# METHODS-Group/ProximalGalerkin

Measured on AMD Instinct MI355X. Metric: proximal-Newton iterations/sec, 2048^2 P1 obstacle (LVPP Newton inner loop), higher is better.
Workload: dtype f64; 1 GPU; 2048x2048 right-diagonal P1 obstacle problem on [-1,1]^2, phi_set obstacle, f=0, settings B: alpha double_exponential, alpha_max 100, tol 0.0001; snes_rtol 1e-6, Newton linear solves to true relative residual 1e-10; mixed_unknowns=8396802, step=one full LVPP solve from the zero state, parallelism=single

## Files before the change

proximalgalerkin_amd/csrc/pgx_api.hip:

```cpp
#include <algorithm>
#include <atomic>
#include <chrono>
#include <thread>
#include <cmath>
#include <cstdio>
#include <cstring>
#include <deque>
#include <map>
#include <mutex>
#include <string>
#include <vector>

#include "../../include/pgx.h"
#include "../../include/pgx_nd.h"
#include "pgx_comm.h"
#include "pgx_internal.h"

static thread_local std::string g_create_error;

struct DistLevel {
  int g, glo, H, ghi;
};
struct Dist {
  bool on = false;
// ... 105 lines not shown
  int xcd_remap = 2;
  int tail_verts = 1100;
  int spmv_stream = 1;
  int nu_coarse = 0;
  int fused_k3 = 1;
  int fused_legs = 1;
  int fused_min = 4000;
  int cgs_selective = 1;
  long cgs_skipped = 0, cgs_total = 0;
  double cgs_eta2 = 1e-4;
  TailArgs tail{};
  pgx_nd* lu = nullptr;
  pgx_comm* lu_comm = nullptr;
  double* Jmix = nullptr;
  bool dh_interior = false;
  int stag_its = 12;
  double stag_gain = 1e-4;
  int smooth_d32 = 0;
  int k6_max = 0;
  int mg_f32 = 1;
  int f32_min = 4000;
  int f32_k6_max = 4300000;
  int f32_rr_max = 300000;
  int resid_grid = 1;
  int spmv_stencil = 1;
  bool lu_active = false;
  bool check_replicas = false;
  double *obs_partials = nullptr, *d_out6 = nullptr;
  int obs_blocks = 0;
  bool prof = false;
// ... 978 lines not shown
  if (!h->patch_f32) h->patch_sym = 0;
  if (h->patch_f32 == 2 && !h->patch_sym) h->patch_f32 = 1;
  if (const char* e = pgx_tune("PGX_P2_FALLBACK_ITS")) h->p2_fallback_its = std::max(1, atoi(e));
  {
    const char* e = pgx_tune("PGX_TAIL2");
    pgxk_mg_tail_select(e ? atoi(e) : 1);
  }
  if (const char* e = pgx_tune("PGX_FUSED_LEGS")) h->fused_legs = atoi(e);
  if (const char* e = pgx_tune("PGX_FUSED_K3")) h->fused_k3 = atoi(e);
  if (const char* e = pgx_tune("PGX_NU_COARSE")) h->nu_coarse = atoi(e);
  if (const char* e = pgx_tune("PGX_SPMV_STREAM")) h->spmv_stream = atoi(e);
  if (const char* e = pgx_tune("PGX_SPMV_BAL")) h->spmv_bal = atoi(e);
  if (const char* e = pgx_tune("PGX_SPMV_DICT")) h->spmv_dict = atoi(e);
  if (const char* e = pgx_tune("PGX_SPMV_STENCIL")) h->spmv_stencil = atoi(e);
  if (const char* e = pgx_tune("PGX_RESID_GRID")) h->resid_grid = atoi(e);
  if (const char* e = pgx_tune("PGX_K6_MAX")) h->k6_max = atoi(e);
  if (const char* e = pgx_tune("PGX_SMOOTH_D32")) h->smooth_d32 = atoi(e);
  if (const char* e = pgx_tune("PGX_HOST_POLL")) h->host_poll = atoi(e);
  if (const char* e = pgx_tune("PGX_GS_WIDE")) h->gs_wide = atoi(e) >= 16 ? 16 : 8;
  if (const char* e = pgx_tune("PGX_FUSED_PUBLISH")) h->fused_publish = atoi(e);
  if (const char* e = pgx_tune("PGX_FUSED_RESID")) h->fused_resid = atoi(e);
  if (const char* e = pgx_tune("PGX_LEAN_RHS")) h->lean_rhs = atoi(e);
  if (const char* e = pgx_tune("PGX_FUSED_STEP")) h->fused_step = atoi(e);
  if (const char* e = pgx_tune("PGX_LAZY_NORM")) h->lazy_norm = atoi(e);
  if (const char* e = pgx_tune("PGX_V_F32")) h->v_f32 = atoi(e);
  if (const char* e = pgx_tune("PGX_V_F32_GAIN")) h->v_f32_gain = atof(e);
  if (const char* e = pgx_tune("PGX_V_F32_MAX")) h->v_f32_max = atof(e);
  if (const char* e = pgx_tune("PGX_V_F32_MIN")) h->v_f32_min = atoi(e);
  if (const char* e = pgx_tune("PGX_Z_F32")) h->z_f32 = atoi(e);
  if (const char* e = pgx_tune("PGX_F32_DBF16")) h->f32_dbf16 = atoi(e);
// ... 501 lines not shown
    const int rc = allreduce_dev(h, h->d_small, 1);
    if (rc) return rc;
  }
  {
    const int rc = replica_agree(h, h->d_small, 1);
    if (rc) return rc;
  }
  {
    const int rc = fetch_small(h, h->d_small, 1);
    if (rc) return rc;
  }
  *out = std::sqrt(h->h_small[0]);
  return PGX_OK;
}

static void residual_dev(pgx_handle* h, const double* x, double* F, int with_d = 0) {
  PhaseTimer t(h, 0);
  if (h->degree == 2) {
    pgxk_residual_p2_cells(h->st, h->nc, h->nd, h->cdofs, h->coords, h->mask, h->gbc, x, h->xk, h->alpha, h->f, h->q2,
                           h->p2_v2c_ptr, h->p2_v2c_ent, h->p2_stash, F, h->geoq);
    pgxk_residual_final(h->st, h->nd, h->mask, h->gbc, h->bphi, x, F);
    return;
  }
  if (h->resid_grid && h->structured && !h->lev.empty() && h->lev[0].uniform) {
    pgxk_resid_fill_grid(h->st, with_d ? 1 : 0, h->lev[0], h->fill_lds, h->rowptr, h->v2c_ptr, h->v2c_ent, h->v2c_pos, h->cells,
                         h->coords, h->mask, h->gbc, h->bphi, x, h->xk, h->alpha, h->f, h->q, F, h->Dv, with_d);
    h->dh_interior = with_d != 0;
    if (with_d == 2) h->dv_lean = true;
    if (with_d == 1) h->dv_lean = false;
    return;
  }
  pgxk_resid_fill_p1(h->st, with_d, h->n, h->fill_lds, h->rowptr, h->v2c_ptr, h->v2c_ent, h->v2c_pos, h->cells,
                     h->coords, h->mask, h->gbc, h->bphi, x, h->xk, h->alpha, h->f, h->q, F, h->Dv, h->geoq);
}

static int jacobian_dev(pgx_handle* h, const double* x, bool have_d = false) {
  if (!(have_d && h->degree == 1)) {
    PhaseTimer t(h, 1);
    if (h->degree == 2) {
      pgxk_fill_rows_p2(h->st, 2, h->nd, h->s_fill_lds, h->s_rowptr, h->p2_v2c_ptr, h->p2_v2c_ent, h->p2_v2c_pos,
                        h->cdofs, h->coords, x + h->nd, h->q2, h->s_D, h->geoq);
      pgxk_fill_rows_p1_Dp2(h->st, h->n, h->fill_lds, h->rowptr, h->v2c_ptr, h->v2c_ent, h->v2c_pos, h->cdofs, h->coords,
                            x + h->nd, h->q2, h->Dv, h->geoq);
    } else if (h->resid_grid && h->structured && !h->lev.empty() && h->lev[0].uniform) {
      pgxk_resid_fill_grid(h->st, 1, h->lev[0], h->fill_lds, h->rowptr, h->v2c_ptr, h->v2c_ent, h->v2c_pos, h->cells, h->coords,
                           h->mask, h->gbc, h->bphi, x, h->xk, h->alpha, h->f, h->q, h->w, h->Dv, 1);
      h->dh_interior = true;
      h->dv_lean = false;
      have_d = true;
    } else {
      pgxk_fill_rows(h->st, 2, h->n, h->fill_lds, h->rowptr, h->v2c_ptr, h->v2c_ent, h->v2c_pos, h->cells, h->coords,
                     x + h->n, h->q, h->Dv, h->geoq);
    }
  }
  if (h->structured) {
    PhaseTimer t(h, 2);
    pgxk_csr_to_stencil_h(h->st, h->n, h->nx + 1, h->rowptr, h->colm, h->Dv, h->lev[0].Dh,
                          (have_d && h->degree == 1 && h->dh_interior) ? h->lev[0].ny : 0);
    h->dh_interior = false;
    if (h->lev[0].Dh32) pgxk_to_float(h->st, (size_t)4 * h->n, h->lev[0].Dh, h->lev[0].Dh32);
    if (h->lev[0].f32) pgxk_f_pack_d(h->st, h->lev[0]);
    if (h->lev[0].Dd4) pgxk_pack_d4(h->st, h->lev[0]);
    const int ld = h->dist.on ? h->dist.ldist : 0;
    for (size_t l = 1; l < h->lev.size(); ++l) {
      if (h->dist.on && (int)l == ld) {
        const Dist& D = h->dist;
        const GridLevel& G = h->lev[l];
#ifdef PGX_DSTEN_FLOAT
        h->err = "PGX_DSTEN_FLOAT builds do not support sharded handles";
        return PGX_EINVAL;
#else
        pgxk_rap7h(h->st, h->lev[l - 1], h->lev[l - 1].Dh, D.view, D.view_S);
        pgxk_view_to_global(h->st, 4, D.view.n, G.n, G.nx + 1, D.view_row0, D.view_own0, D.view_H, D.view_S, G.Dh);
        const int rc = allreduce_dev(h, G.Dh, (size_t)4 * G.n);
        if (rc) return rc;
#endif
      } else {
        pgxk_rap7h(h->st, h->lev[l - 1], h->lev[l - 1].Dh, h->lev[l], h->lev[l].Dh);
      }
      if (h->lev[l].f32) pgxk_f_pack_d(h->st, h->lev[l]);
    }
  }
  h->jac_valid = true;
  h->patch_fresh = false;
  h->p2st.fresh = false;
  return PGX_OK;
}

static bool p2st_ready(pgx_handle* h) {
  pgx_handle::P2St& S = h->p2st;
  if (S.state == 0 || !S.select || (h->dist.on && !S.dist_enable) || !h->s_K || !h->s_D) return false;
  static const int nt[4] = {19, 9, 9, 9}, off[4] = {0, 19, 28, 37};
  const size_t G = (size_t)h->n;
// ... 1464 lines not shown
```

proximalgalerkin_amd/csrc/pgx_internal.h:

```cpp
#pragma once
#include <hip/hip_runtime.h>
#include <stdint.h>
#include <stddef.h>

#include "pgx_scope.h"

#ifdef PGX_DSTEN_FLOAT
typedef float dsten_t;
#else
typedef double dsten_t;
#endif

#define PGX_MAX_NQ 16
#define PGX_BLOCK 256
#ifndef PGX_TILE_X
#define PGX_TILE_X 32
#define PGX_TILE_Y 16
#endif
#ifndef PGX_ROWMAP_TY
#define PGX_ROWMAP_TY 16
#endif
#ifndef PGX_ROWMAP_BLOCK
#define PGX_ROWMAP_BLOCK 512
#endif
// ... 18 lines not shown
  double *xu, *xp, *xu2, *xp2;
  double *bu, *bp;
  double *ru, *rp;
  int f32;
  double4* Dd4;
  void* Dq;
  int dbf16;
  float2 *xf, *xf2, *bf;
};

struct StConst {
  double K[7], M[7];
  int uniform;
};

#define PGX_TAIL_MAX 8
#define PGX_TAIL_VERTS 17000
struct TailLevel {
  int nx, ny, n;
  int interior_free;
  double ic[8];
  const double *K, *M;
  const dsten_t* Dh;
  StConst sc;
  const uint8_t* mask;
  double *xu, *xp, *xu2, *xp2, *bu, *bp, *ru, *rp;
};
struct TailArgs {
  int nlev, nu, coarse_sweeps;
  double alpha, omega;
// ... 33 lines not shown
                       double* out, const PgxDotScale* scale = nullptr, int wide = 8);
int pgxk_multidot_blocks(size_t len);
int pgxk_stream_blocks(size_t len);
void pgxk_reduce_publish(hipStream_t st, int nb, const double* partials, int nrows, double* out, double* hout, int n1, const double* src1,
                         double* dst1, unsigned long long seq, unsigned long long* seqp);
int pgxk_axpy_norms(hipStream_t st, size_t len, const double* x, double* y, double* partials);
void pgxk_multiaxpy(hipStream_t st, size_t len, int nv, const double* V, size_t ldv, const double* h, double* w);
void pgxk_lincomb(hipStream_t st, size_t len, int nv, const double* Z, size_t ldz, const double* y, double* x,
                  int accumulate);

void pgxk_csr_to_stencil(hipStream_t st, int n, int sx, const int32_t* rowptr, const int32_t* colm, const double* vals,
                         double* S);
void pgxk_csr_to_stencil_h(hipStream_t st, int n, int sx, const int32_t* rowptr, const int32_t* colm,
                           const double* vals, dsten_t* Sh, int frame_ny = 0);
void pgxk_rap7(hipStream_t st, const GridLevel& f, const double* Sf, const GridLevel& c, double* Sc);
void pgxk_rap7h(hipStream_t st, const GridLevel& f, const dsten_t* Sfh, const GridLevel& c, dsten_t* Sch);
void pgxk_st_apply(hipStream_t st, int mode, const GridLevel& L, double alpha, const double* xu, const double* xp,
                   const double* bu, const double* bp, double omega, int first, double* yu, double* yp);
void pgxk_restrict(hipStream_t st, const GridLevel& f, const double* ru, const double* rp, const GridLevel& c,
                   double* bu, double* bp);
void pgxk_prolong_add(hipStream_t st, const GridLevel& c, const double* cu, const double* cp, const GridLevel& f,
                      double* xu, double* xp);
void pgxk_coarse_mask(hipStream_t st, const GridLevel& c, uint8_t* mask_c, const GridLevel& f);
void pgxk_view_to_global(hipStream_t st, int ns, int n_view, int n_glob, int sx, int row0, int own0, int nown,
                         const double* in, double* out);
void pgxk_st_smooth2(hipStream_t st, int post, const GridLevel& L, double alpha, const double* xu, const double* xp,
                     const GridLevel* C, const double* cu, const double* cp, const double* bu, const double* bp,
                     double omega, int remap, double* yu, double* yp);
void pgxk_st_spmv(hipStream_t st, const GridLevel& L, double alpha, const double* xu, const double* xp, int remap, double* yu,
                  double* yp, const float2* xf = nullptr ,
                  const double* bu = nullptr, const double* bp = nullptr, double s = 1.0 );
// ... 69 lines not shown
void pgxk_p2st_pack(hipStream_t st, int nx, int nv, int i0, int ni, int j0, int nj, size_t G, const int32_t* rowptr, const double* D,
                    void* Dst, int f32);
void pgxk_p2st_check(hipStream_t st, const P2StTab& S, int nx, int nv, int i0, int ni, int j0, int nj, double alpha_ref, double tol,
                     const int32_t* rowptr, const double* K, const double* M, int* fail);
void pgxk_p2_rows_csr(hipStream_t st, int nrows, const int32_t* rows, const int32_t* rowptr, const int32_t* colm, const double* K,
                      const double* M, const double* D, double alpha, const uint8_t* mask, const double* xu, const double* xp,
                      const double* bu, const double* bp, double* yu, double* yp);
void pgxk_resid_fill_p1(hipStream_t st, int write_d, int n, size_t lds_bytes, const int32_t* rowptr,
                        const int32_t* v2c_ptr, const int32_t* v2c_ent, const int32_t* v2c_pos, const int32_t* cells,
                        const double* coords, const uint8_t* mask, const double* gbc, const double* bphi,
                        const double* x, const double* xk, double alpha, double f, QuadTab q, double* F, double* Dout,
                        const double* geo = nullptr);
void pgxk_resid_fill_grid(hipStream_t st, int write_d, const GridLevel& L, size_t lds_bytes, const int32_t* rowptr,
                          const int32_t* v2c_ptr, const int32_t* v2c_ent, const int32_t* v2c_pos, const int32_t* cells,
                          const double* coords, const uint8_t* mask, const double* gbc, const double* bphi, const double* x,
                          const double* xk, double alpha, double f, QuadTab q, double* F, double* Dout, int write_sh);
void pgxk_axpy_dot(hipStream_t st, size_t len, int nv, const double* V, size_t ldv, const double* h1, double* w,
                   double* partials, double* out);
void pgxk_multiaxpy_scale(hipStream_t st, size_t len, int nv, const double* V, size_t ldv, const double* h,
                          double scale, double* w);
void pgxk_multiaxpy_norm(hipStream_t st, size_t len, int nv, const double* V, size_t ldv, const double* h, double* w,
                         double* partials, double* out, int wide = 8);
void pgxk_multiaxpy_norm_f32(hipStream_t st, size_t len, int nv, const float* V, size_t ldv, const double* h, int from_vnext, double* w,
                             float* vnext, double* partials, double* out, int wide = 8);
void pgxk_f_pack_d(hipStream_t st, const GridLevel& L);
void pgxk_f_smooth(hipStream_t st, int K, int first, const GridLevel& L, double alpha, const float2* xf, const double* b64u,
                   const double* b64p, const GridLevel* C, const float2* cf, const double* cdu, const double* cdp, double omega,
                   int remap, float2* yf, double* y64u, double* y64p, float2* cbf = nullptr, double* cb64u = nullptr,
                   double* cb64p = nullptr, double bscale = 1.0,
                   const float* b32u = nullptr, const float* b32p = nullptr);
void pgxk_f_resid_restrict(hipStream_t st, const GridLevel& L, double alpha, const float2* xf, const GridLevel& C, int remap,
// ... 6 lines not shown
```

proximalgalerkin_amd/csrc/pgx_kernels.hip:

```cpp
#include "pgx_internal.h"
#include "pgx_stencil.h"
#include <algorithm>
#include <type_traits>

#define WAVE 64

static bool first_use_on_device(int slot) {
  static bool done[4][64] = {};
  int dev = 0;
  if (hipGetDevice(&dev) != hipSuccess || dev < 0 || dev >= 64) return true;
  if (done[slot][dev]) return false;
  done[slot][dev] = true;
  return true;
}

__device__ __forceinline__ double wave_sum(double v) {
#pragma unroll
  for (int o = WAVE / 2; o > 0; o >>= 1) v += __shfl_xor(v, o, WAVE);
  return v;
}

__device__ __forceinline__ double2 ldnt2(const double2* p) {
  typedef double v2d __attribute__((ext_vector_type(2)));
  const v2d v = __builtin_nontemporal_load((const v2d*)p);
// ... 418 lines not shown
      for (int k = rowptr[i]; k < rowptr[i + 1]; ++k) Dout[k] = row[k - rowptr[i]];
  }
  if (WRITE_D && !FRAME) {
    __syncthreads();
    for (int k = threadIdx.x; k < len; k += PGX_BLOCK) Dout[base + k] = acc[k];
  }
}

#define PGX_RF_TX 32
#define PGX_RF_TY 12
template <bool WRITE_D>
__global__ void __launch_bounds__(PGX_RF_TX * PGX_RF_TY) k_resid_fill_grid(
    int nx, int ny, int n, const int32_t* __restrict__ rowptr, const double* __restrict__ coords, const uint8_t* __restrict__ mask,
    const double* __restrict__ gbc, const double* __restrict__ bphi, const double* __restrict__ x, const double* __restrict__ xk,
    double alpha, double f, QuadTab q, StConst sc, double* __restrict__ F, double* __restrict__ Dout,
    dsten_t* __restrict__ Sh) {
  constexpr int TX = PGX_RF_TX, TY = PGX_RF_TY, IW = TX + 2, IH = TY + 2, SW = TX + 1, SH = TY + 1;
  __shared__ double iu[IH * IW], ip[IH * IW], idp[IH * IW];
  __shared__ double E[2 * SW * SH][6];
  const int sx = nx + 1;
  const int ntx = (nx - 1 + TX - 1) / TX;
  const int i1 = 1 + ((int)blockIdx.x % ntx) * TX, j1 = 1 + ((int)blockIdx.x / ntx) * TY;
  const int tid = threadIdx.x;
  for (int t = tid; t < IH * IW; t += TX * TY) {
    const int gi = i1 - 1 + t % IW, gj = j1 - 1 + t / IW;
    double u = 0.0, p = 0.0, dp = 0.0;
    if (gi <= nx && gj <= ny) {
      const int v = gj * sx + gi;
      u = mask[v] ? gbc[v] : x[v];
      p = x[n + v];
      dp = p - xk[n + v];
// ... 46 lines not shown
      double* d = Dout + rowptr[v];
      d[0] = dSW;
      d[1] = dS;
      d[2] = dW;
      d[3] = dC;
      d[4] = dE;
      d[5] = dN;
      d[6] = dNE;
    }
    if (Sh) {
      Sh[v] = (dsten_t)dC;
      Sh[(size_t)n + v] = (dsten_t)dE;
      Sh[2 * (size_t)n + v] = (dsten_t)dN;
      Sh[3 * (size_t)n + v] = (dsten_t)dNE;
    }
  }
  const int o = (lj + 1) * IW + li + 1;
  const int off[7] = {0, 1, -1, IW, -IW, IW + 1, -IW - 1};
  double Ku = 0.0, Mdp = 0.0, Mu = 0.0;
#pragma unroll
  for (int t = 0; t < 7; ++t) {
    Ku += sc.K[t] * iu[o + off[t]];
    Mdp += sc.M[t] * idp[o + off[t]];
    Mu += sc.M[t] * iu[o + off[t]];
  }
  const double load = adet * 2.0 * (q.mref[0] + q.mref[1] + q.mref[2]);
  F[v] = mask[v] ? x[v] - gbc[v] : alpha * Ku + Mdp - alpha * f * load;
  F[n + v] = Mu - (((dSW + dS) + (dW + dC)) + ((dE + dN) + dNE)) - bphi[v];
}

void pgxk_resid_fill_p1(hipStream_t st, int write_d, int n, size_t lds_bytes, const int32_t* rowptr,
                        const int32_t* v2c_ptr, const int32_t* v2c_ent, const int32_t* v2c_pos, const int32_t* cells,
                        const double* coords, const uint8_t* mask, const double* gbc, const double* bphi,
                        const double* x, const double* xk, double alpha, double f, QuadTab q, double* F, double* Dout,
                        const double* geo) {
  dim3 grid((n + PGX_BLOCK - 1) / PGX_BLOCK), block(PGX_BLOCK);
  if (geo) {
    if (write_d)
      hipLaunchKernelGGL((k_resid_fill_p1_c<true>), grid, block, lds_bytes, st, n, rowptr, v2c_ptr, v2c_ent, v2c_pos, cells, mask, gbc,
                         bphi, x, xk, alpha, f, q, F, Dout, geo);
    else
      hipLaunchKernelGGL((k_resid_fill_p1_c<false>), grid, block, lds_bytes, st, n, rowptr, v2c_ptr, v2c_ent, v2c_pos, cells, mask, gbc,
                         bphi, x, xk, alpha, f, q, F, Dout, geo);
    return;
  }
  if (write_d)
    hipLaunchKernelGGL((k_resid_fill_p1<true, false>), grid, block, lds_bytes, st, n, rowptr, v2c_ptr, v2c_ent, v2c_pos, cells,
                       coords, mask, gbc, bphi, x, xk, alpha, f, q, 0, 0, F, Dout);
  else
    hipLaunchKernelGGL((k_resid_fill_p1<false, false>), grid, block, lds_bytes, st, n, rowptr, v2c_ptr, v2c_ent, v2c_pos, cells,
                       coords, mask, gbc, bphi, x, xk, alpha, f, q, 0, 0, F, Dout);
}

void pgxk_resid_fill_grid(hipStream_t st, int write_d, const GridLevel& L, size_t lds_bytes, const int32_t* rowptr,
                          const int32_t* v2c_ptr, const int32_t* v2c_ent, const int32_t* v2c_pos, const int32_t* cells,
                          const double* coords, const uint8_t* mask, const double* gbc, const double* bphi, const double* x,
                          const double* xk, double alpha, double f, QuadTab q, double* F, double* Dout, int write_sh) {
  const int n = L.n, sx = L.nx + 1;
  dim3 grid((n + PGX_BLOCK - 1) / PGX_BLOCK), block(PGX_BLOCK);
  if (write_d)
    hipLaunchKernelGGL((k_resid_fill_p1<true, true>), grid, block, lds_bytes, st, n, rowptr, v2c_ptr, v2c_ent, v2c_pos, cells,
                       coords, mask, gbc, bphi, x, xk, alpha, f, q, sx, L.ny, F, Dout);
  else
    hipLaunchKernelGGL((k_resid_fill_p1<false, true>), grid, block, lds_bytes, st, n, rowptr, v2c_ptr, v2c_ent, v2c_pos, cells,
                       coords, mask, gbc, bphi, x, xk, alpha, f, q, sx, L.ny, F, Dout);
  if (L.nx < 2 || L.ny < 2) return;
  const int ntx = (L.nx - 1 + PGX_RF_TX - 1) / PGX_RF_TX, nty = (L.ny - 1 + PGX_RF_TY - 1) / PGX_RF_TY;
  const StConst sc = make_stconst(L);
  if (write_d)
    hipLaunchKernelGGL(k_resid_fill_grid<true>, dim3(ntx * nty), dim3(PGX_RF_TX * PGX_RF_TY), 0, st, L.nx, L.ny, n, rowptr, coords,
                       mask, gbc, bphi, x, xk, alpha, f, q, sc, F, write_sh == 2 ? nullptr : Dout, write_sh ? L.Dh : nullptr);
  else
    hipLaunchKernelGGL(k_resid_fill_grid<false>, dim3(ntx * nty), dim3(PGX_RF_TX * PGX_RF_TY), 0, st, L.nx, L.ny, n, rowptr, coords,
                       mask, gbc, bphi, x, xk, alpha, f, q, sc, F, Dout, nullptr);
}

void pgxk_fill_rows(hipStream_t st, int mode, int n, size_t lds_bytes, const int32_t* rowptr, const int32_t* v2c_ptr,
                    const int32_t* v2c_ent, const int32_t* v2c_pos, const int32_t* cells, const double* coords,
                    const double* psi, QuadTab q, double* out, const double* geo) {
  dim3 grid((n + PGX_BLOCK - 1) / PGX_BLOCK), block(PGX_BLOCK);
  if (geo) {
    if (mode == 0)
      hipLaunchKernelGGL(k_fill_rows_c<0>, grid, block, lds_bytes, st, n, rowptr, v2c_ptr, v2c_ent, v2c_pos, cells, psi, q, out, geo);
    else if (mode == 1)
      hipLaunchKernelGGL(k_fill_rows_c<1>, grid, block, lds_bytes, st, n, rowptr, v2c_ptr, v2c_ent, v2c_pos, cells, psi, q, out, geo);
    else
      hipLaunchKernelGGL(k_fill_rows_c<2>, grid, block, lds_bytes, st, n, rowptr, v2c_ptr, v2c_ent, v2c_pos, cells, psi, q, out, geo);
    return;
  }
// ... 1110 lines not shown
    const double v = vals[k];
    if (o == 0) s[0] = v;
    else if (o == 1) s[1] = v;
    else if (o == sx) s[2] = v;
    else if (o == sx + 1) s[3] = v;
  }
#pragma unroll
  for (int k = 0; k < 4; ++k) Sh[(size_t)k * n + i] = (dsten_t)s[k];
}
void pgxk_csr_to_stencil_h(hipStream_t st, int n, int sx, const int32_t* rowptr, const int32_t* colm,
                           const double* vals, dsten_t* Sh, int frame_ny) {
  hipLaunchKernelGGL(k_csr_to_stencil_h, dim3((n + PGX_BLOCK - 1) / PGX_BLOCK), dim3(PGX_BLOCK), 0, st, n, sx, rowptr,
                     colm, vals, Sh, frame_ny);
}

__global__ void __launch_bounds__(PGX_BLOCK) k_rap7h(int nxf, int nyf, int nf, const dsten_t* __restrict__ Sfh, int nxc,
                                                     int nyc, int ncv, dsten_t* __restrict__ Sch) {
  const int C = blockIdx.x * blockDim.x + threadIdx.x;
  if (C >= ncv) return;
  constexpr int OX[7] = {0, 1, -1, 0, 0, 1, -1};
  constexpr int OY[7] = {0, 0, 0, 1, -1, 1, -1};
  constexpr int KEEP[4] = {0, 1, 3, 5};
  const int sxc = nxc + 1, sxf = nxf + 1;
  const int I = C % sxc, Jc = C / sxc;
  double out[4] = {0, 0, 0, 0};
#pragma unroll
  for (int oa = 0; oa < 7; ++oa) {
    const int ax = 2 * I + OX[oa], ay = 2 * Jc + OY[oa];
    if (ax < 0 || ax > nxf || ay < 0 || ay > nyf) continue;
    const double wa = pw(OX[oa], OY[oa]);
    const int a = ay * sxf + ax;
    double cf[7];
    ld7h(Sfh, nf, sxf, a, ax, ay, nxf, nyf, cf);
#pragma unroll
    for (int os = 0; os < 7; ++os) {
      const double coef = wa * cf[os];
      const int dx = OX[oa] + OX[os], dy = OY[oa] + OY[os];
#pragma unroll
      for (int q = 0; q < 4; ++q) {
        const double w2 = pw(dx - 2 * OX[KEEP[q]], dy - 2 * OY[KEEP[q]]);
        if (w2 != 0.0) out[q] += coef * w2;
      }
    }
  }
#pragma unroll
  for (int q = 0; q < 4; ++q) {
    const int nx_ = I + OX[KEEP[q]], ny_ = Jc + OY[KEEP[q]];
    const bool ok = nx_ >= 0 && nx_ <= nxc && ny_ >= 0 && ny_ <= nyc;
    Sch[(size_t)q * ncv + C] = (dsten_t)(ok ? out[q] : 0.0);
  }
}
void pgxk_rap7h(hipStream_t st, const GridLevel& f, const dsten_t* Sfh, const GridLevel& c, dsten_t* Sch) {
  hipLaunchKernelGGL(k_rap7h, dim3((c.n + PGX_BLOCK - 1) / PGX_BLOCK), dim3(PGX_BLOCK), 0, st, f.nx, f.ny, f.n, Sfh,
                     c.nx, c.ny, c.n, Sch);
}

__global__ void k_coarse_mask(int nxc, int nyc, int ncv, int nxf, const uint8_t* __restrict__ mf,
                              uint8_t* __restrict__ mc) {
  const int C = blockIdx.x * blockDim.x + threadIdx.x;
  if (C >= ncv) return;
  const int I = C % (nxc + 1), J = C / (nxc + 1);
  mc[C] = mf[(size_t)(2 * J) * (nxf + 1) + 2 * I];
}
void pgxk_coarse_mask(hipStream_t st, const GridLevel& c, uint8_t* mask_c, const GridLevel& f) {
  hipLaunchKernelGGL(k_coarse_mask, dim3((c.n + PGX_BLOCK - 1) / PGX_BLOCK), dim3(PGX_BLOCK), 0, st, c.nx, c.ny, c.n,
                     f.nx, f.mask, mask_c);
}

__global__ void __launch_bounds__(PGX_BLOCK) k_view_to_global(int ns, int n_view, int n_glob, int sx, int row0,
// ... 1829 lines not shown
```

proximalgalerkin_amd/csrc/pgx_mg32.hip:

```cpp
#include <algorithm>

#include "pgx_internal.h"
#include "pgx_stencil.h"

#define F32_BLOCK 512
#ifndef F32_LEAN
#define F32_LEAN 0
#endif
#ifndef F32_WAVES_EU
#define F32_WAVES_EU 2
#endif
#ifndef F32_K6_SPLIT
#define F32_K6_SPLIT 0
#endif
#ifndef F32_K6_TY_TOP
#define F32_K6_TY_TOP 20
#endif
#define F32_RR_CYB 2
#define F32_TB 2
__host__ __device__ constexpr int f32_tb(int K, int RR) { return (K == 6 && !RR) ? 4 : F32_TB; }

__device__ __forceinline__ float lane_shr1f(float x) {
  int v = __float_as_int(x);
  v = __builtin_amdgcn_update_dpp(v, v, 0x138, 0xf, 0xf, false);
  return __int_as_float(v);
}

typedef float f_v2f __attribute__((ext_vector_type(2)));
typedef __bf16 f_v2bf __attribute__((ext_vector_type(2)));
__device__ __forceinline__ uint32_t f_pack_bf16x2(float lo, float hi) {
  const f_v2f f = {lo, hi};
  return __builtin_bit_cast(uint32_t, __builtin_convertvector(f, f_v2bf));
}
__device__ __forceinline__ void f_pack_d(float4 q, float4& out) { out = q; }
__device__ __forceinline__ void f_pack_d(float4 q, uint2& out) { out = make_uint2(f_pack_bf16x2(q.x, q.y), f_pack_bf16x2(q.z, q.w)); }
__device__ __forceinline__ float4 f_unpack_d(float4 q) { return q; }
__device__ __forceinline__ float4 f_unpack_d(uint2 w) {
  return make_float4(__uint_as_float(w.x << 16), __uint_as_float(w.x & 0xffff0000u), __uint_as_float(w.y << 16),
                     __uint_as_float(w.y & 0xffff0000u));
}
__device__ __forceinline__ void f_zero_d(float4& q) { q = make_float4(0.f, 0.f, 0.f, 0.f); }
__device__ __forceinline__ void f_zero_d(uint2& w) { w = make_uint2(0u, 0u); }

template <class DT>
__global__ void __launch_bounds__(256) k_f_pack_d(int n, const dsten_t* __restrict__ Dh, DT* __restrict__ Dq) {
  const int v = blockIdx.x * blockDim.x + threadIdx.x;
  if (v >= n) return;
  const float big = 1e30f;
  f_pack_d(make_float4(fminf((float)Dh[v], big), fminf((float)Dh[(size_t)n + v], big), fminf((float)Dh[2 * (size_t)n + v], big),
                       fminf((float)Dh[3 * (size_t)n + v], big)),
           Dq[v]);
}
void pgxk_f_pack_d(hipStream_t st, const GridLevel& L) {
  if (L.dbf16)
    hipLaunchKernelGGL(k_f_pack_d<uint2>, dim3((L.n + 255) / 256), dim3(256), 0, st, L.n, L.Dh, (uint2*)L.Dq);
  else
    hipLaunchKernelGGL(k_f_pack_d<float4>, dim3((L.n + 255) / 256), dim3(256), 0, st, L.n, L.Dh, (float4*)L.Dq);
}

struct FCoef {
  float kv[7], mv[7], dv[7];
  int rowbc;
};
struct FConst {
  float kc[7], mc[7];
  float k0, k1, k3, k5, m0, m1, m3, m5;
// ... 1116 lines not shown
```

Before: 151.4 Newton iterations/s.

## Write fine-level stencil and packed copies directly from residual fill; LDS-staged RAP

When enabled (default on for structured uniform single-GPU P1), the grid residual/fill kernel writes the fine stencil Dh plus its double4 and f32/bf16 packed copies directly. A new frame-only kernel handles boundary vertices, replacing the full-mesh CSR fill pass. This skips the separate csr_to_stencil, f_pack_d and pack_d4 passes on the fine level. The Galerkin RAP kernel also emits packed coarse copies inline, and on large coarse levels stages the fine stencil in LDS tiles, removing the per-level pack launches and redundant global loads. Costs are more register and store pressure in the fused kernels and a more complex code path.

```diff
diff --git a/proximalgalerkin_amd/csrc/pgx_api.hip b/proximalgalerkin_amd/csrc/pgx_api.hip
--- a/proximalgalerkin_amd/csrc/pgx_api.hip
+++ b/proximalgalerkin_amd/csrc/pgx_api.hip
@@ -143,6 +143,9 @@
   pgx_comm* lu_comm = nullptr;
   double* Jmix = nullptr;
   bool dh_interior = false;
+  int d_direct = 1;
+  int rap_lds_min = 60000;
+  bool d0_direct = false;
   int stag_its = 12;
   double stag_gain = 1e-4;
   int smooth_d32 = 0;
@@ -1151,6 +1154,8 @@
   if (const char* e = pgx_tune("PGX_SPMV_DICT")) h->spmv_dict = atoi(e);
   if (const char* e = pgx_tune("PGX_SPMV_STENCIL")) h->spmv_stencil = atoi(e);
   if (const char* e = pgx_tune("PGX_RESID_GRID")) h->resid_grid = atoi(e);
+  if (const char* e = pgx_tune("PGX_D_DIRECT")) h->d_direct = atoi(e);
+  if (const char* e = pgx_tune("PGX_RAP_LDS_MIN")) h->rap_lds_min = atoi(e);
   if (const char* e = pgx_tune("PGX_K6_MAX")) h->k6_max = atoi(e);
   if (const char* e = pgx_tune("PGX_SMOOTH_D32")) h->smooth_d32 = atoi(e);
   if (const char* e = pgx_tune("PGX_HOST_POLL")) h->host_poll = atoi(e);
@@ -1682,6 +1687,11 @@
   return PGX_OK;
 }
 
+static bool d_direct_on(const pgx_handle* h) {
+  return h->d_direct && !h->dist.on && h->degree == 1 && h->structured && h->resid_grid && !h->lev.empty() && h->lev[0].uniform &&
+         sizeof(dsten_t) == 8 && !h->lev[0].Dh32;
+}
+
 static void residual_dev(pgx_handle* h, const double* x, double* F, int with_d = 0) {
   PhaseTimer t(h, 0);
   if (h->degree == 2) {
@@ -1692,8 +1702,9 @@
   }
   if (h->resid_grid && h->structured && !h->lev.empty() && h->lev[0].uniform) {
     pgxk_resid_fill_grid(h->st, with_d ? 1 : 0, h->lev[0], h->fill_lds, h->rowptr, h->v2c_ptr, h->v2c_ent, h->v2c_pos, h->cells,
-                         h->coords, h->mask, h->gbc, h->bphi, x, h->xk, h->alpha, h->f, h->q, F, h->Dv, with_d);
+                         h->coords, h->mask, h->gbc, h->bphi, x, h->xk, h->alpha, h->f, h->q, F, h->Dv, with_d, d_direct_on(h), h->colm);
     h->dh_interior = with_d != 0;
+    h->d0_direct = with_d != 0 && d_direct_on(h);
     if (with_d == 2) h->dv_lean = true;
     if (with_d == 1) h->dv_lean = false;
     return;
@@ -1712,8 +1723,9 @@
                             x + h->nd, h->q2, h->Dv, h->geoq);
     } else if (h->resid_grid && h->structured && !h->lev.empty() && h->lev[0].uniform) {
       pgxk_resid_fill_grid(h->st, 1, h->lev[0], h->fill_lds, h->rowptr, h->v2c_ptr, h->v2c_ent, h->v2c_pos, h->cells, h->coords,
-                           h->mask, h->gbc, h->bphi, x, h->xk, h->alpha, h->f, h->q, h->w, h->Dv, 1);
+                           h->mask, h->gbc, h->bphi, x, h->xk, h->alpha, h->f, h->q, h->w, h->Dv, 1, d_direct_on(h), h->colm);
       h->dh_interior = true;
+      h->d0_direct = d_direct_on(h);
       h->dv_lean = false;
       have_d = true;
     } else {
@@ -1723,12 +1735,16 @@
   }
   if (h->structured) {
     PhaseTimer t(h, 2);
-    pgxk_csr_to_stencil_h(h->st, h->n, h->nx + 1, h->rowptr, h->colm, h->Dv, h->lev[0].Dh,
-                          (have_d && h->degree == 1 && h->dh_interior) ? h->lev[0].ny : 0);
+    const bool direct = d_direct_on(h);
+    const bool d0 = direct && have_d && h->dh_interior && h->d0_direct;
+    if (!d0)
+      pgxk_csr_to_stencil_h(h->st, h->n, h->nx + 1, h->rowptr, h->colm, h->Dv, h->lev[0].Dh,
+                            (have_d && h->degree == 1 && h->dh_interior) ? h->lev[0].ny : 0);
     h->dh_interior = false;
+    h->d0_direct = false;
     if (h->lev[0].Dh32) pgxk_to_float(h->st, (size_t)4 * h->n, h->lev[0].Dh, h->lev[0].Dh32);
-    if (h->lev[0].f32) pgxk_f_pack_d(h->st, h->lev[0]);
-    if (h->lev[0].Dd4) pgxk_pack_d4(h->st, h->lev[0]);
+    if (h->lev[0].f32 && !d0) pgxk_f_pack_d(h->st, h->lev[0]);
+    if (h->lev[0].Dd4 && !d0) pgxk_pack_d4(h->st, h->lev[0]);
     const int ld = h->dist.on ? h->dist.ldist : 0;
     for (size_t l = 1; l < h->lev.size(); ++l) {
       if (h->dist.on && (int)l == ld) {
@@ -1744,7 +1760,8 @@
         if (rc) return rc;
 #endif
       } else {
-        pgxk_rap7h(h->st, h->lev[l - 1], h->lev[l - 1].Dh, h->lev[l], h->lev[l].Dh);
+        pgxk_rap7h(h->st, h->lev[l - 1], h->lev[l - 1].Dh, h->lev[l], h->lev[l].Dh, direct, direct && h->lev[l].n >= h->rap_lds_min);
+        if (direct) continue;
       }
       if (h->lev[l].f32) pgxk_f_pack_d(h->st, h->lev[l]);
     }
diff --git a/proximalgalerkin_amd/csrc/pgx_internal.h b/proximalgalerkin_amd/csrc/pgx_internal.h
--- a/proximalgalerkin_amd/csrc/pgx_internal.h
+++ b/proximalgalerkin_amd/csrc/pgx_internal.h
@@ -56,6 +56,20 @@
   int uniform;
 };
 
+typedef float f_v2f __attribute__((ext_vector_type(2)));
+typedef __bf16 f_v2bf __attribute__((ext_vector_type(2)));
+__device__ __forceinline__ uint32_t f_pack_bf16x2(float lo, float hi) {
+  const f_v2f f = {lo, hi};
+  return __builtin_bit_cast(uint32_t, __builtin_convertvector(f, f_v2bf));
+}
+__device__ __forceinline__ void f_pack_d(float4 q, float4& out) { out = q; }
+__device__ __forceinline__ void f_pack_d(float4 q, uint2& out) { out = make_uint2(f_pack_bf16x2(q.x, q.y), f_pack_bf16x2(q.z, q.w)); }
+template <class DT>
+__device__ __forceinline__ void f_pack_dq(dsten_t d0, dsten_t d1, dsten_t d2, dsten_t d3, DT& out) {
+  const float big = 1e30f;
+  f_pack_d(make_float4(fminf((float)d0, big), fminf((float)d1, big), fminf((float)d2, big), fminf((float)d3, big)), out);
+}
+
 #define PGX_TAIL_MAX 8
 #define PGX_TAIL_VERTS 17000
 struct TailLevel {
@@ -119,7 +133,7 @@
 void pgxk_csr_to_stencil_h(hipStream_t st, int n, int sx, const int32_t* rowptr, const int32_t* colm,
                            const double* vals, dsten_t* Sh, int frame_ny = 0);
 void pgxk_rap7(hipStream_t st, const GridLevel& f, const double* Sf, const GridLevel& c, double* Sc);
-void pgxk_rap7h(hipStream_t st, const GridLevel& f, const dsten_t* Sfh, const GridLevel& c, dsten_t* Sch);
+void pgxk_rap7h(hipStream_t st, const GridLevel& f, const dsten_t* Sfh, const GridLevel& c, dsten_t* Sch, int pack = 0, int staged = 0);
 void pgxk_st_apply(hipStream_t st, int mode, const GridLevel& L, double alpha, const double* xu, const double* xp,
                    const double* bu, const double* bp, double omega, int first, double* yu, double* yp);
 void pgxk_restrict(hipStream_t st, const GridLevel& f, const double* ru, const double* rp, const GridLevel& c,
@@ -219,7 +233,8 @@
 void pgxk_resid_fill_grid(hipStream_t st, int write_d, const GridLevel& L, size_t lds_bytes, const int32_t* rowptr,
                           const int32_t* v2c_ptr, const int32_t* v2c_ent, const int32_t* v2c_pos, const int32_t* cells,
                           const double* coords, const uint8_t* mask, const double* gbc, const double* bphi, const double* x,
-                          const double* xk, double alpha, double f, QuadTab q, double* F, double* Dout, int write_sh);
+                          const double* xk, double alpha, double f, QuadTab q, double* F, double* Dout, int write_sh,
+                          int direct = 0, const int32_t* colm = nullptr);
 void pgxk_axpy_dot(hipStream_t st, size_t len, int nv, const double* V, size_t ldv, const double* h1, double* w,
                    double* partials, double* out);
 void pgxk_multiaxpy_scale(hipStream_t st, size_t len, int nv, const double* V, size_t ldv, const double* h,
diff --git a/proximalgalerkin_amd/csrc/pgx_kernels.hip b/proximalgalerkin_amd/csrc/pgx_kernels.hip
--- a/proximalgalerkin_amd/csrc/pgx_kernels.hip
+++ b/proximalgalerkin_amd/csrc/pgx_kernels.hip
@@ -456,7 +456,7 @@
     int nx, int ny, int n, const int32_t* __restrict__ rowptr, const double* __restrict__ coords, const uint8_t* __restrict__ mask,
     const double* __restrict__ gbc, const double* __restrict__ bphi, const double* __restrict__ x, const double* __restrict__ xk,
     double alpha, double f, QuadTab q, StConst sc, double* __restrict__ F, double* __restrict__ Dout,
-    dsten_t* __restrict__ Sh) {
+    dsten_t* __restrict__ Sh, double4* __restrict__ Dd4, void* __restrict__ Dq, int dbf16) {
   constexpr int TX = PGX_RF_TX, TY = PGX_RF_TY, IW = TX + 2, IH = TY + 2, SW = TX + 1, SH = TY + 1;
   __shared__ double iu[IH * IW], ip[IH * IW], idp[IH * IW];
   __shared__ double E[2 * SW * SH][6];
@@ -533,6 +533,13 @@
       Sh[2 * (size_t)n + v] = (dsten_t)dN;
       Sh[3 * (size_t)n + v] = (dsten_t)dNE;
     }
+    if (Dd4) Dd4[v] = make_double4(dC, dE, dN, dNE);
+    if (Dq) {
+      if (dbf16)
+        f_pack_dq((dsten_t)dC, (dsten_t)dE, (dsten_t)dN, (dsten_t)dNE, ((uint2*)Dq)[v]);
+      else
+        f_pack_dq((dsten_t)dC, (dsten_t)dE, (dsten_t)dN, (dsten_t)dNE, ((float4*)Dq)[v]);
+    }
   }
   const int o = (lj + 1) * IW + li + 1;
   const int off[7] = {0, 1, -1, IW, -IW, IW + 1, -IW - 1};
@@ -546,6 +553,98 @@
   const double load = adet * 2.0 * (q.mref[0] + q.mref[1] + q.mref[2]);
   F[v] = mask[v] ? x[v] - gbc[v] : alpha * Ku + Mdp - alpha * f * load;
   F[n + v] = Mu - (((dSW + dS) + (dW + dC)) + ((dE + dN) + dNE)) - bphi[v];
+}
+
+#define PGX_FRAME_BLOCK 64
+template <bool WRITE_D>
+__global__ void __launch_bounds__(PGX_FRAME_BLOCK) k_resid_fill_frame(
+    int nx, int ny, int n, const int32_t* __restrict__ rowptr, const int32_t* __restrict__ colm, const int32_t* __restrict__ v2c_ptr,
+    const int32_t* __restrict__ v2c_ent, const int32_t* __restrict__ v2c_pos, const int32_t* __restrict__ cells,
+    const double* __restrict__ coords, const uint8_t* __restrict__ mask, const double* __restrict__ gbc,
+    const double* __restrict__ bphi, const double* __restrict__ x, const double* __restrict__ xk, double alpha, double f, QuadTab q,
+    double* __restrict__ F, double* __restrict__ Dout, dsten_t* __restrict__ Sh, double4* __restrict__ Dd4, void* __restrict__ Dq,
+    int dbf16) {
+  __shared__ double acc[PGX_FRAME_BLOCK * 7];
+  const int sx = nx + 1;
+  const int t = blockIdx.x * PGX_FRAME_BLOCK + threadIdx.x;
+  if (t >= 2 * sx + 2 * (ny - 1)) return;
+  int gi, gj;
+  if (t < sx) {
+    gi = t, gj = 0;
+  } else if (t < 2 * sx) {
+    gi = t - sx, gj = ny;
+  } else if (t < 2 * sx + ny - 1) {
+    gi = 0, gj = 1 + t - 2 * sx;
+  } else {
+    gi = nx, gj = 1 + t - 2 * sx - (ny - 1);
+  }
+  const int i = gj * sx + gi;
+  double* row = acc + threadIdx.x * 7;
+  const int r0 = rowptr[i], rl = min(rowptr[i + 1] - r0, 7);
+  if (WRITE_D)
+    for (int k = 0; k < rl; ++k) row[k] = 0.0;
+  double Fu = 0.0, Fp = 0.0;
+  const int ke = v2c_ptr[i + 1];
+  for (int k = v2c_ptr[i]; k < ke; ++k) {
+    const int e = v2c_ent[k];
+    const int c = e >> 2, a = e & 3;
+    const int v[3] = {cells[3 * c], cells[3 * c + 1], cells[3 * c + 2]};
+    const P1Geom g = p1_geom(coords[2 * v[0]], coords[2 * v[0] + 1], coords[2 * v[1]], coords[2 * v[1] + 1],
+                             coords[2 * v[2]], coords[2 * v[2] + 1]);
+    double u[3], p[3], dp[3];
+#pragma unroll
+    for (int b = 0; b < 3; ++b) {
+      u[b] = mask[v[b]] ? gbc[v[b]] : x[v[b]];
+      p[b] = x[n + v[b]];
+      dp[b] = p[b] - xk[n + v[b]];
+    }
+    double d[3] = {0.0, 0.0, 0.0};
+    for (int k2 = 0; k2 < q.nq; ++k2) {
+      const double pq = p[0] * q.N[k2][0] + p[1] * q.N[k2][1] + p[2] * q.N[k2][2];
+      const double wa = q.w[k2] * exp(pq) * q.N[k2][a];
+      d[0] += wa * q.N[k2][0];
+      d[1] += wa * q.N[k2][1];
+      d[2] += wa * q.N[k2][2];
+    }
+    const double gx = u[0] * g.G[0][0] + u[1] * g.G[1][0] + u[2] * g.G[2][0];
+    const double gy = u[0] * g.G[0][1] + u[1] * g.G[1][1] + u[2] * g.G[2][1];
+    const double Ku = 0.5 * g.adet * (g.G[a][0] * gx + g.G[a][1] * gy);
+    const double Mdp = g.adet * (q.Mref[a][0] * dp[0] + q.Mref[a][1] * dp[1] + q.Mref[a][2] * dp[2]);
+    const double Mu = g.adet * (q.Mref[a][0] * u[0] + q.Mref[a][1] * u[1] + q.Mref[a][2] * u[2]);
+    Fu += alpha * Ku + Mdp - alpha * f * g.adet * q.mref[a];
+    Fp += Mu - g.adet * (d[0] + d[1] + d[2]);
+    if (WRITE_D) {
+      const int pos = v2c_pos[k];
+      row[min(pos & 0xff, 6)] += g.adet * d[0];
+      row[min((pos >> 8) & 0xff, 6)] += g.adet * d[1];
+      row[min((pos >> 16) & 0xff, 6)] += g.adet * d[2];
+    }
+  }
+  F[i] = mask[i] ? x[i] - gbc[i] : Fu;
+  F[n + i] = Fp - bphi[i];
+  if (WRITE_D) {
+    double s[4] = {0, 0, 0, 0};
+    for (int k = 0; k < rl; ++k) {
+      const double val = row[k];
+      Dout[r0 + k] = val;
+      const int o = (colm[r0 + k] & 0x7fffffff) - i;
+      if (o == 0) s[0] = val;
+      else if (o == 1) s[1] = val;
+      else if (o == sx) s[2] = val;
+      else if (o == sx + 1) s[3] = val;
+    }
+    if (Sh) {
+#pragma unroll
+      for (int k = 0; k < 4; ++k) Sh[(size_t)k * n + i] = (dsten_t)s[k];
+      if (Dd4) Dd4[i] = make_double4(s[0], s[1], s[2], s[3]);
+      if (Dq) {
+        if (dbf16)
+          f_pack_dq((dsten_t)s[0], (dsten_t)s[1], (dsten_t)s[2], (dsten_t)s[3], ((uint2*)Dq)[i]);
+        else
+          f_pack_dq((dsten_t)s[0], (dsten_t)s[1], (dsten_t)s[2], (dsten_t)s[3], ((float4*)Dq)[i]);
+      }
+    }
+  }
 }
 
 void pgxk_resid_fill_p1(hipStream_t st, int write_d, int n, size_t lds_bytes, const int32_t* rowptr,
@@ -574,24 +673,40 @@
 void pgxk_resid_fill_grid(hipStream_t st, int write_d, const GridLevel& L, size_t lds_bytes, const int32_t* rowptr,
                           const int32_t* v2c_ptr, const int32_t* v2c_ent, const int32_t* v2c_pos, const int32_t* cells,
                           const double* coords, const uint8_t* mask, const double* gbc, const double* bphi, const double* x,
-                          const double* xk, double alpha, double f, QuadTab q, double* F, double* Dout, int write_sh) {
+                          const double* xk, double alpha, double f, QuadTab q, double* F, double* Dout, int write_sh, int direct,
+                          const int32_t* colm) {
   const int n = L.n, sx = L.nx + 1;
-  dim3 grid((n + PGX_BLOCK - 1) / PGX_BLOCK), block(PGX_BLOCK);
-  if (write_d)
-    hipLaunchKernelGGL((k_resid_fill_p1<true, true>), grid, block, lds_bytes, st, n, rowptr, v2c_ptr, v2c_ent, v2c_pos, cells,
-                       coords, mask, gbc, bphi, x, xk, alpha, f, q, sx, L.ny, F, Dout);
-  else
-    hipLaunchKernelGGL((k_resid_fill_p1<false, true>), grid, block, lds_bytes, st, n, rowptr, v2c_ptr, v2c_ent, v2c_pos, cells,
-                       coords, mask, gbc, bphi, x, xk, alpha, f, q, sx, L.ny, F, Dout);
+  const bool copies = direct && write_d && write_sh && colm;
+  double4* Dd4 = copies ? L.Dd4 : nullptr;
+  void* Dq = copies && L.f32 ? L.Dq : nullptr;
+  if (direct && colm) {
+    const int nframe = 2 * sx + 2 * (L.ny - 1);
+    dim3 grid((nframe + PGX_FRAME_BLOCK - 1) / PGX_FRAME_BLOCK), block(PGX_FRAME_BLOCK);
+    if (write_d)
+      hipLaunchKernelGGL(k_resid_fill_frame<true>, grid, block, 0, st, L.nx, L.ny, n, rowptr, colm, v2c_ptr, v2c_ent, v2c_pos, cells,
+                         coords, mask, gbc, bphi, x, xk, alpha, f, q, F, Dout, copies ? L.Dh : nullptr, Dd4, Dq, L.dbf16);
+    else
+      hipLaunchKernelGGL(k_resid_fill_frame<false>, grid, block, 0, st, L.nx, L.ny, n, rowptr, colm, v2c_ptr, v2c_ent, v2c_pos, cells,
+                         coords, mask, gbc, bphi, x, xk, alpha, f, q, F, Dout, nullptr, nullptr, nullptr, 0);
+  } else {
+    dim3 grid((n + PGX_BLOCK - 1) / PGX_BLOCK), block(PGX_BLOCK);
+    if (write_d)
+      hipLaunchKernelGGL((k_resid_fill_p1<true, true>), grid, block, lds_bytes, st, n, rowptr, v2c_ptr, v2c_ent, v2c_pos, cells,
+                         coords, mask, gbc, bphi, x, xk, alpha, f, q, sx, L.ny, F, Dout);
+    else
+      hipLaunchKernelGGL((k_resid_fill_p1<false, true>), grid, block, lds_bytes, st, n, rowptr, v2c_ptr, v2c_ent, v2c_pos, cells,
+                         coords, mask, gbc, bphi, x, xk, alpha, f, q, sx, L.ny, F, Dout);
+  }
   if (L.nx < 2 || L.ny < 2) return;
   const int ntx = (L.nx - 1 + PGX_RF_TX - 1) / PGX_RF_TX, nty = (L.ny - 1 + PGX_RF_TY - 1) / PGX_RF_TY;
   const StConst sc = make_stconst(L);
   if (write_d)
     hipLaunchKernelGGL(k_resid_fill_grid<true>, dim3(ntx * nty), dim3(PGX_RF_TX * PGX_RF_TY), 0, st, L.nx, L.ny, n, rowptr, coords,
-                       mask, gbc, bphi, x, xk, alpha, f, q, sc, F, write_sh == 2 ? nullptr : Dout, write_sh ? L.Dh : nullptr);
+                       mask, gbc, bphi, x, xk, alpha, f, q, sc, F, write_sh == 2 ? nullptr : Dout, write_sh ? L.Dh : nullptr, Dd4, Dq,
+                       L.dbf16);
   else
     hipLaunchKernelGGL(k_resid_fill_grid<false>, dim3(ntx * nty), dim3(PGX_RF_TX * PGX_RF_TY), 0, st, L.nx, L.ny, n, rowptr, coords,
-                       mask, gbc, bphi, x, xk, alpha, f, q, sc, F, Dout, nullptr);
+                       mask, gbc, bphi, x, xk, alpha, f, q, sc, F, Dout, nullptr, nullptr, nullptr, 0);
 }
 
 void pgxk_fill_rows(hipStream_t st, int mode, int n, size_t lds_bytes, const int32_t* rowptr, const int32_t* v2c_ptr,
@@ -1732,24 +1847,19 @@
                      colm, vals, Sh, frame_ny);
 }
 
-__global__ void __launch_bounds__(PGX_BLOCK) k_rap7h(int nxf, int nyf, int nf, const dsten_t* __restrict__ Sfh, int nxc,
-                                                     int nyc, int ncv, dsten_t* __restrict__ Sch) {
-  const int C = blockIdx.x * blockDim.x + threadIdx.x;
-  if (C >= ncv) return;
+template <class LD>
+__device__ __forceinline__ void rap7h_vertex(LD ld, int I, int Jc, int nxf, int nyf, int nxc, int nyc, dsten_t st4[4]) {
   constexpr int OX[7] = {0, 1, -1, 0, 0, 1, -1};
   constexpr int OY[7] = {0, 0, 0, 1, -1, 1, -1};
   constexpr int KEEP[4] = {0, 1, 3, 5};
-  const int sxc = nxc + 1, sxf = nxf + 1;
-  const int I = C % sxc, Jc = C / sxc;
   double out[4] = {0, 0, 0, 0};
 #pragma unroll
   for (int oa = 0; oa < 7; ++oa) {
     const int ax = 2 * I + OX[oa], ay = 2 * Jc + OY[oa];
     if (ax < 0 || ax > nxf || ay < 0 || ay > nyf) continue;
     const double wa = pw(OX[oa], OY[oa]);
-    const int a = ay * sxf + ax;
     double cf[7];
-    ld7h(Sfh, nf, sxf, a, ax, ay, nxf, nyf, cf);
+    ld(ax, ay, cf);
 #pragma unroll
     for (int os = 0; os < 7; ++os) {
       const double coef = wa * cf[os];
@@ -1765,12 +1875,95 @@
   for (int q = 0; q < 4; ++q) {
     const int nx_ = I + OX[KEEP[q]], ny_ = Jc + OY[KEEP[q]];
     const bool ok = nx_ >= 0 && nx_ <= nxc && ny_ >= 0 && ny_ <= nyc;
-    Sch[(size_t)q * ncv + C] = (dsten_t)(ok ? out[q] : 0.0);
-  }
-}
-void pgxk_rap7h(hipStream_t st, const GridLevel& f, const dsten_t* Sfh, const GridLevel& c, dsten_t* Sch) {
+    st4[q] = (dsten_t)(ok ? out[q] : 0.0);
+  }
+}
+__device__ __forceinline__ void rap7h_store(const dsten_t st4[4], int ncv, int C, dsten_t* Sch, void* Dq, int dbf16) {
+#pragma unroll
+  for (int q = 0; q < 4; ++q) Sch[(size_t)q * ncv + C] = st4[q];
+  if (Dq) {
+    if (dbf16)
+      f_pack_dq(st4[0], st4[1], st4[2], st4[3], ((uint2*)Dq)[C]);
+    else
+      f_pack_dq(st4[0], st4[1], st4[2], st4[3], ((float4*)Dq)[C]);
+  }
+}
+
+__global__ void __launch_bounds__(PGX_BLOCK) k_rap7h(int nxf, int nyf, int nf, const dsten_t* __restrict__ Sfh, int nxc,
+                                                     int nyc, int ncv, dsten_t* __restrict__ Sch, void* __restrict__ Dq, int dbf16) {
+  const int C = blockIdx.x * blockDim.x + threadIdx.x;
+  if (C >= ncv) return;
+  const int sxc = nxc + 1, sxf = nxf + 1;
+  const int I = C % sxc, Jc = C / sxc;
+  dsten_t st4[4];
+  rap7h_vertex([&](int ax, int ay, double cf[7]) { ld7h(Sfh, nf, sxf, ay * sxf + ax, ax, ay, nxf, nyf, cf); }, I, Jc, nxf, nyf, nxc,
+               nyc, st4);
+  rap7h_store(st4, ncv, C, Sch, Dq, dbf16);
+}
+
+#define PGX_RAPL_CX 32
+#define PGX_RAPL_CY 8
+__global__ void __launch_bounds__(PGX_RAPL_CX * PGX_RAPL_CY) k_rap7h_lds(int nxf, int nyf, int nf, const dsten_t* __restrict__ Sfh,
+                                                                         int nxc, int nyc, int ncv, dsten_t* __restrict__ Sch,
+                                                                         void* __restrict__ Dq, int dbf16) {
+  constexpr int CX = PGX_RAPL_CX, CY = PGX_RAPL_CY, FW = 2 * CX + 2, FH = 2 * CY + 2, HW = FW / 2;
+  constexpr int NT = CX * CY, NV = FH * FW, IT = (NV + NT - 1) / NT;
+  __shared__ dsten_t s[4][NV];
+  const int sxc = nxc + 1, sxf = nxf + 1;
+  const int ntx = (sxc + CX - 1) / CX;
+  const int I0 = ((int)blockIdx.x % ntx) * CX, J0 = ((int)blockIdx.x / ntx) * CY;
+  const int fx0 = 2 * I0 - 2, fy0 = 2 * J0 - 2;
+  dsten_t val[IT][4];
+#pragma unroll
+  for (int k = 0; k < IT; ++k) {
+    const int t = (int)threadIdx.x + k * NT, ly = t / FW, lx = t % FW;
+    const int fx = fx0 + lx, fy = fy0 + ly;
+    val[k][0] = val[k][1] = val[k][2] = val[k][3] = 0;
+    if (t < NV && fx >= 0 && fx <= nxf && fy >= 0 && fy <= nyf) {
+      const size_t a = (size_t)fy * sxf + fx;
+#pragma unroll
+      for (int sl = 0; sl < 4; ++sl) val[k][sl] = Sfh[(size_t)sl * nf + a];
+    }
+  }
+#pragma unroll
+  for (int k = 0; k < IT; ++k) {
+    const int t = (int)threadIdx.x + k * NT, ly = t / FW, lx = t % FW;
+    if (t < NV) {
+#pragma unroll
+      for (int sl = 0; sl < 4; ++sl) s[sl][ly * FW + (lx & 1) * HW + (lx >> 1)] = val[k][sl];
+    }
+  }
+  __syncthreads();
+  const int I = I0 + (int)threadIdx.x % CX, Jc = J0 + (int)threadIdx.x / CX;
+  if (I > nxc || Jc > nyc) return;
+  auto at = [&](int lx, int ly) { return ly * FW + (lx & 1) * HW + (lx >> 1); };
+  dsten_t st4[4];
+  rap7h_vertex(
+      [&](int ax, int ay, double cf[7]) {
+        const int lx = ax - fx0, ly = ay - fy0;
+        const int l = at(lx, ly), lw = at(lx - 1, ly), ls = at(lx, ly - 1), lsw = at(lx - 1, ly - 1);
+        cf[0] = s[0][l];
+        cf[1] = (ax < nxf) ? s[1][l] : 0.0;
+        cf[2] = (ax > 0) ? s[1][lw] : 0.0;
+        cf[3] = (ay < nyf) ? s[2][l] : 0.0;
+        cf[4] = (ay > 0) ? s[2][ls] : 0.0;
+        cf[5] = (ax < nxf && ay < nyf) ? s[3][l] : 0.0;
+        cf[6] = (ax > 0 && ay > 0) ? s[3][lsw] : 0.0;
+      },
+      I, Jc, nxf, nyf, nxc, nyc, st4);
+  rap7h_store(st4, ncv, Jc * sxc + I, Sch, Dq, dbf16);
+}
+
+void pgxk_rap7h(hipStream_t st, const GridLevel& f, const dsten_t* Sfh, const GridLevel& c, dsten_t* Sch, int pack, int staged) {
+  void* Dq = (pack && c.f32) ? c.Dq : nullptr;
+  if (staged) {
+    const int ntx = (c.nx + 1 + PGX_RAPL_CX - 1) / PGX_RAPL_CX, nty = (c.ny + 1 + PGX_RAPL_CY - 1) / PGX_RAPL_CY;
+    hipLaunchKernelGGL(k_rap7h_lds, dim3(ntx * nty), dim3(PGX_RAPL_CX * PGX_RAPL_CY), 0, st, f.nx, f.ny, f.n, Sfh, c.nx, c.ny, c.n, Sch,
+                       Dq, c.dbf16);
+    return;
+  }
   hipLaunchKernelGGL(k_rap7h, dim3((c.n + PGX_BLOCK - 1) / PGX_BLOCK), dim3(PGX_BLOCK), 0, st, f.nx, f.ny, f.n, Sfh,
-                     c.nx, c.ny, c.n, Sch);
+                     c.nx, c.ny, c.n, Sch, Dq, c.dbf16);
 }
 
 __global__ void k_coarse_mask(int nxc, int nyc, int ncv, int nxf, const uint8_t* __restrict__ mf,
diff --git a/proximalgalerkin_amd/csrc/pgx_mg32.hip b/proximalgalerkin_amd/csrc/pgx_mg32.hip
--- a/proximalgalerkin_amd/csrc/pgx_mg32.hip
+++ b/proximalgalerkin_amd/csrc/pgx_mg32.hip
@@ -26,14 +26,6 @@
   return __int_as_float(v);
 }
 
-typedef float f_v2f __attribute__((ext_vector_type(2)));
-typedef __bf16 f_v2bf __attribute__((ext_vector_type(2)));
-__device__ __forceinline__ uint32_t f_pack_bf16x2(float lo, float hi) {
-  const f_v2f f = {lo, hi};
-  return __builtin_bit_cast(uint32_t, __builtin_convertvector(f, f_v2bf));
-}
-__device__ __forceinline__ void f_pack_d(float4 q, float4& out) { out = q; }
-__device__ __forceinline__ void f_pack_d(float4 q, uint2& out) { out = make_uint2(f_pack_bf16x2(q.x, q.y), f_pack_bf16x2(q.z, q.w)); }
 __device__ __forceinline__ float4 f_unpack_d(float4 q) { return q; }
 __device__ __forceinline__ float4 f_unpack_d(uint2 w) {
   return make_float4(__uint_as_float(w.x << 16), __uint_as_float(w.x & 0xffff0000u), __uint_as_float(w.y << 16),
@@ -46,10 +38,7 @@
 __global__ void __launch_bounds__(256) k_f_pack_d(int n, const dsten_t* __restrict__ Dh, DT* __restrict__ Dq) {
   const int v = blockIdx.x * blockDim.x + threadIdx.x;
   if (v >= n) return;
-  const float big = 1e30f;
-  f_pack_d(make_float4(fminf((float)Dh[v], big), fminf((float)Dh[(size_t)n + v], big), fminf((float)Dh[2 * (size_t)n + v], big),
-                       fminf((float)Dh[3 * (size_t)n + v], big)),
-           Dq[v]);
+  f_pack_dq(Dh[v], Dh[(size_t)n + v], Dh[2 * (size_t)n + v], Dh[3 * (size_t)n + v], Dq[v]);
 }
 void pgxk_f_pack_d(hipStream_t st, const GridLevel& L) {
   if (L.dbf16)
```

Result: faster. 155.3 Newton iterations/s (median of 6 runs) (+2.6%).
